# wbuntine/libstb

Hardware: AMD Instinct MI355X
Metric: S-table cells/s (higher is better)
Workload: dtype f64

## Files before the change

### include/stb_hip.h

```cpp
#ifndef STB_HIP_H
#define STB_HIP_H

#include <stddef.h>
#include <stdint.h>

#ifdef __cplusplus
extern "C" {
#endif

const char *stb_last_error(void);
int stb_device_count(void);
int stb_device_name(char *buf, int len);

int stb_set_device(int dev);
int stb_get_device(void);
int stb_device_enter(int dev);
void stb_device_leave(int prev);

void *stb_device_malloc(size_t bytes);
void stb_device_free(void *p);
void *stb_host_malloc(size_t bytes);
void stb_host_free(void *p);
void *stb_host_malloc_huge(size_t bytes);
void stb_host_free_huge(void *p);
// ... 16 lines not shown
uint64_t stb_vrowoff(unsigned n, unsigned M);

void stb_extend_policy(unsigned usedN, unsigned usedM, unsigned maxN, unsigned maxM, int N, int M,
                       unsigned *newN, unsigned *newM);

#define STB_FILL_SCALED 0
#define STB_FILL_LOGDOMAIN 1
#define STB_FILL_SCALED_STEP 2
#define STB_FILL_SPLIT 3
#define STB_FILL_FUSED 4
#define STB_FILL_PC 5
#define STB_FILL_CHAIN 6
#define STB_FILL_CHAINX 7
#define STB_FILL_CK 8
#define STB_FILL_HB 9
size_t stb_fill_workspace_bytes(unsigned N, unsigned M, int D);
int stb_default_variant(void);
int stb_fill_S(const double *a_host, int D, unsigned N, unsigned M, double *d_tables,
               uint64_t table_stride, double *d_S1, uint64_t s1_stride, void *d_ws, size_t ws_bytes,
               int variant, void *stream);
int stb_fill_tuning(unsigned N, unsigned M, int D, int *C_out, int *R_out, int *launches);
int stb_fill_status(void);
unsigned stb_fill_fallbacks(void);
unsigned stb_slow_launches(void);
int stb_shared_gpu_mode(void);
void stb_set_shared_gpu(int mode);
void stb_note_launch_span(double span_ms, double expect_ms);
int stb_has_ablation(void);
void stb_pool_trim(void);
void stb_fill_profile_begin(void);
int stb_fill_profile_end(double *kernel_ms_total, int *launches);
double stb_fill_profile_span(void);
int stb_fill_V(const double *a_host, int D, unsigned N, unsigned M, double *d_vtables,
               uint64_t vtable_stride, void *d_ws, size_t ws_bytes, void *stream);
int stb_fill_V_exact(const double *a_host, int D, unsigned N, unsigned M, double *d_vtables,
                     uint64_t vtable_stride, void *d_ws, size_t ws_bytes, void *stream);

int stb_fill_takes_kind(unsigned N, unsigned M, int D, int kind);
int stb_fill_Sf(const double *a_host, int D, unsigned N, unsigned M, float *d_tables, uint64_t table_stride,
                double *d_S1, uint64_t s1_stride, void *d_ws, size_t ws_bytes, void *stream);
int stb_fill_Vf(const double *a_host, int D, unsigned N, unsigned M, float *d_vtables, uint64_t vtable_stride,
                void *d_ws, size_t ws_bytes, void *stream);

int stb_table_to_float(const double *d_src, float *d_dst, uint64_t elems, void *stream);

int stb_lookup_S(const double *d_table, const double *d_S1, unsigned N, unsigned M,
// ... 120 lines not shown
```

### libstb_amd/capi.py

```python
from __future__ import annotations

import ctypes as C
import os
from functools import lru_cache

import numpy as np

_HERE = os.path.dirname(os.path.abspath(__file__))
LIB_PATH = os.environ.get("STB_LIB_PATH") or os.path.join(_HERE, "lib", "libstb_amd.so")

S_STABLE, S_UVTABLE, S_FLOAT, S_VERBOSE, S_QUITONBOUND, S_THREADS, S_ASYMPT = 1, 2, 4, 8, 16, 32, 64
FILL_SCALED, FILL_LOGDOMAIN, FILL_SCALED_STEP, FILL_SPLIT, FILL_FUSED, FILL_PC, FILL_CHAIN, FILL_CHAINX, FILL_CK, FILL_HB = 0, 1, 2, 3, 4, 5, 6, 7, 8, 9

c_double_p = C.POINTER(C.c_double)
c_u32_p = C.POINTER(C.c_uint32)
c_u16_p = C.POINTER(C.c_uint16)
c_int_p = C.POINTER(C.c_int)
c_float_p = C.POINTER(C.c_float)

LOGDENS = C.CFUNCTYPE(C.c_double, C.c_double, C.c_void_p)
GETVAL = C.CFUNCTYPE(None, c_u32_p, c_u16_p, C.c_uint, C.c_uint)


class StbError(RuntimeError):
    pass


@lru_cache(maxsize=None)
def lib() -> C.CDLL:
    if not os.path.exists(LIB_PATH):
        raise StbError(
            f"{LIB_PATH} is missing: build it with `python -c 'import __graft_entry__ as g; g.build()'` "
            "or `make -C libstb_amd/csrc` (there is no pure-Python or CPU implementation)")
    try:
        import torch
    except Exception:
        pass
    L = C.CDLL(LIB_PATH)
    u, d, i, vp, u64, sz = C.c_uint, C.c_double, C.c_int, C.c_void_p, C.c_uint64, C.c_size_t

    ROUND5 = {"stb_groups_pairs_begin", "stb_groups_pairs_put", "stb_groups_pairs_put_ragged", "stb_groups_pairs_commit",
              "stb_groups_update_pairs", "stb_groups_fallbacks", "stb_grid_shape", "stb_bterms_update",
              "stb_table_probe", "stb_slow_launches", "stb_shared_gpu_mode", "stb_set_shared_gpu", "stb_note_launch_span",
              "stb_lookup_V", "stb_lookup_U", "stb_lookup_UV", "stb_groups_aterms_multi", "stb_groups_create_node",
              "stb_groups_last_form"}

    def sig(name, res, args):
        try:
            f = getattr(L, name)
        except AttributeError:
            if name in ROUND5 and os.environ.get("STB_LIB_PATH"):
                return
            raise
        f.restype = res
        f.argtypes = args

    sig("S_make", vp, [u, u, u, u, d, C.c_uint32])
    sig("S_tag", None, [vp, C.c_char_p])
    sig("S_remake", i, [vp, d])
    sig("S_free", None, [vp])
    for n in ("S_S", "S_U", "S_UV", "S_V", "S_asympt"):
        sig(n, d, [vp, u, u])
    sig("S_S1", d, [vp, u])
    sig("S_report", None, [vp, vp])
    sig("stb_extend_policy", None, [u, u, u, u, i, i, C.POINTER(u), C.POINTER(u)])
    sig("stb_table_sync", i, [vp])
    sig("stb_table_probe", None, [vp, i, C.POINTER(u), C.POINTER(u), sz, c_double_p])
    sig("stb_table_mirrored", None, [vp, C.POINTER(u), C.POINTER(u)])
# ... 3 lines not shown
    sig("stb_device_count", i, [])
    sig("stb_device_name", i, [C.c_char_p, i])
    sig("stb_set_device", i, [i])
    sig("stb_get_device", i, [])
    sig("stb_device_enter", i, [i])
    sig("stb_device_leave", None, [i])
    sig("stb_device_malloc", vp, [sz])
    sig("stb_device_free", None, [vp])
    sig("stb_host_malloc", vp, [sz])
    sig("stb_host_free", None, [vp])
    sig("stb_memcpy_h2d", i, [vp, vp, sz, vp])
    sig("stb_memcpy_d2h", i, [vp, vp, sz, vp])
    sig("stb_stream_sync", i, [vp])
    for n in ("stb_cells", "stb_elems", "stb_vcells", "stb_velems"):
        sig(n, u64, [u, u])
    sig("stb_rowoff", u64, [u, u])
    sig("stb_vrowoff", u64, [u, u])
    sig("stb_fill_workspace_bytes", sz, [u, u, i])
    sig("stb_default_variant", i, [])
    sig("stb_fill_S", i, [c_double_p, i, u, u, vp, u64, vp, u64, vp, sz, i, vp])
    sig("stb_fill_tuning", i, [u, u, i, c_int_p, c_int_p, c_int_p])
    sig("stb_fill_status", i, [])
    sig("stb_fill_fallbacks", C.c_uint, [])
    sig("stb_has_ablation", i, [])
    sig("stb_slow_launches", C.c_uint, [])
    sig("stb_shared_gpu_mode", i, [])
    sig("stb_set_shared_gpu", None, [i])
    sig("stb_note_launch_span", None, [C.c_double, C.c_double])
    sig("stb_fill_profile_begin", None, [])
    sig("stb_fill_profile_end", i, [c_double_p, c_int_p])
    sig("stb_fill_profile_span", C.c_double, [])
    sig("stb_fill_V", i, [c_double_p, i, u, u, vp, u64, vp, sz, vp])
    sig("stb_fill_V_exact", i, [c_double_p, i, u, u, vp, u64, vp, sz, vp])
    sig("stb_fill_Vf", i, [c_double_p, i, u, u, vp, u64, vp, sz, vp])
    sig("stb_fill_Sf", i, [c_double_p, i, u, u, vp, u64, vp, u64, vp, sz, vp])
    sig("stb_fill_takes_kind", i, [u, u, i, i])
    sig("stb_bterms_create", vp, [c_u32_p, i])
    sig("stb_bterms_update", i, [vp, c_u32_p, i])
    sig("stb_bterms_eval", i, [vp, c_double_p, i, d, d, d, c_double_p])
    sig("stb_bterms_free", None, [vp])
    sig("stb_table_to_float", i, [vp, vp, u64, vp])
    sig("stb_lookup_S", i, [vp, vp, u, u, vp, vp, u64, vp, vp])
    sig("stb_lookup_V", i, [vp, u, u, vp, vp, u64, vp, vp])
    sig("stb_lookup_U", i, [vp, u, u, C.c_double, vp, vp, u64, vp, vp])
    sig("stb_lookup_UV", i, [vp, u, u, C.c_double, vp, vp, u64, vp, vp])
    sig("stb_sweep_workspace_bytes", sz, [u64, i])
# ... 525 lines not shown
```

### libstb_amd/csrc/abi.hip

```cpp

#include <mutex>
#include <vector>

#include "stb_common.h"


static thread_local char g_err[512] = "";

int stb_fail(const char *fmt, ...) {
  va_list ap;
  va_start(ap, fmt);
  vsnprintf(g_err, sizeof(g_err), fmt, ap);
  va_end(ap);
  return 1;
}

extern "C" const char *stb_last_error(void) { return g_err; }

#include <atomic>
static std::atomic<unsigned> g_slow_launches{0};
static std::atomic<int> g_shared_mode{-2};
extern "C" void yaps_message(const char *fmt, ...);

static int shared_mode_now() {
// ... 221 lines not shown
  }
  if (release >= 0) pool_raw_free(p, release);
  return known;
}

extern "C" void stb_pool_trim(void) {
  STB_ENTRY;
  std::vector<pool_block> drop;
  {
    std::lock_guard<std::mutex> lk(g_pool_mu);
    for (size_t i = 0; i < g_pool.size();) {
      if (!g_pool[i].used) {
        drop.push_back(g_pool[i]);
        g_pool.erase(g_pool.begin() + i);
      } else {
        i++;
      }
    }
    g_pool_idle[0] = g_pool_idle[1] = 0;
  }
  for (const pool_block &q : drop) pool_raw_free(q.p, q.kind);
}

extern "C" void *stb_device_malloc(size_t bytes) {
  STB_ENTRY;
  void *p = nullptr;
  hipError_t e = stb_pool_malloc(&p, bytes ? bytes : 1, 0);
  if (e != hipSuccess) {
    stb_fail("hipMalloc(%zu) failed: %s", bytes, hipGetErrorString(e));
    (void)hipGetLastError();
    return nullptr;
  }
  return p;
}
extern "C" void stb_device_free(void *p) {
  STB_ENTRY;
  if (p && !stb_pool_free(p)) (void)hipFree(p);
}
extern "C" void *stb_host_malloc(size_t bytes) {
  STB_ENTRY;
  void *p = nullptr;
  hipError_t e = stb_pool_malloc(&p, bytes ? bytes : 1, 1);
  if (e != hipSuccess) {
    stb_fail("hipHostMalloc(%zu) failed: %s", bytes, hipGetErrorString(e));
    (void)hipGetLastError();
    return nullptr;
// ... 121 lines not shown
```

### libstb_amd/csrc/fill.hip

```cpp

#include "stb_common.h"

static unsigned frontier_pitch(unsigned M) { return (unsigned)stb_align_up((size_t)M + 2, 64); }

int stb_period_rows(unsigned N) {
  int bits = 1;
  while ((1ull << bits) < (unsigned long long)N) bits++;
  const int p = 1450 / (2 * bits + 1);
  return p < 1 ? 1 : p;
}

struct fill_prof {
  bool armed = false;
  int used = 0;
  hipEvent_t ev[2 * 4096];
  int made = 0;
  double span_ms = 0.0;
};
static thread_local fill_prof g_prof;

void stb_prof_events(hipEvent_t *e0, hipEvent_t *e1) {
  *e0 = *e1 = nullptr;
  if (!g_prof.armed || g_prof.used + 2 > 2 * 4096) return;
  while (g_prof.made < g_prof.used + 2) {
// ... 174 lines not shown
  A.H = 256 - 64 * ncw;
  A.R = stb_env_int("STB_FILL_R", A.H);
  if (A.R > A.H) A.R = A.H;
  if (A.R < 1) A.R = 1;
  A.Wv = 256 - A.H;
}

void stb_fill_last(last_fill *out) { *out = g_last; }

int stb_fill_status_of(last_fill *lf) {
  if (!lf->hdr) return 0;
  unsigned h[10] = {0, 0, 0, 0, 0, 0, 0, 0, 0, 0};
  HIPCHK(hipMemcpyAsync(h, lf->hdr, lf->stamped ? sizeof(h) : 4 * sizeof(unsigned), hipMemcpyDeviceToHost, lf->st));
  HIPCHK(hipStreamSynchronize(lf->st));
  if (lf->stamped) {
    const unsigned long long t0 = (unsigned long long)h[STB_HDR_T0] | ((unsigned long long)h[STB_HDR_T0 + 1] << 32);
    const unsigned long long t1 = (unsigned long long)h[STB_HDR_T1] | ((unsigned long long)h[STB_HDR_T1 + 1] << 32);
    if (t0 && t1 > t0)
      stb_note_span((double)(t1 - t0) * 1e-5, 1e-3 * (100.0 + 0.05 * (double)lf->A.N * (1.0 + (double)lf->D / 8.0)), "a table fill (stb_fill_S)");
  }
  if (h[1] == 0) return 0;
  stb_fail("%s: the fill gave up waiting for a neighbour block (code 0x%x, block %u of table %u)",
           lf->s_table ? "stb_fill_S" : "stb_fill_V", h[1], h[2] & 0xffffu, h[2] >> 16);
  if (!lf->can_fall_back || stb_env_int("STB_CHAIN_NO_FALLBACK", 0)) {
    lf->hdr = nullptr;
    return 1;
  }
  lf->hdr = nullptr;
  lf->fell_back = true;
  g_fallbacks++;
  fill_args A = lf->A;
  pc_geometry(A);
  if (stb_launch_pc(A, lf->D, lf->st)) return 1;
  HIPCHK(hipStreamSynchronize(lf->st));
  return 0;
}

extern "C" int stb_fill_status(void) {
  STB_ENTRY;
  return stb_fill_status_of(&g_last);
}

static bool hb_takes_kind(unsigned N, unsigned M, int D, int kind) {
  if (stb_env_int("STB_HB", -1) == 0 || stb_shared_gpu() || !stb_hb_eligible_out(N, M, D, kind)) return false;
  const uint64_t cells = (uint64_t)D * stb_table_cells(N, M);
  if (N < (unsigned)stb_env_int("STB_HB_MIN_N", 512) || cells > (uint64_t)stb_env_int("STB_HB_MAX_MCELLS", 1250) * 1000000ull) return false;
// ... 17 lines not shown
  *D_out = g_a_D;
  g_a_D = 0;
  return true;
}
int stb_a_flush(const fill_args &A, hipStream_t st) {
  stb_a64 av;
  int D = 0;
  if (!stb_a_take(&av, &D)) return 0;
  hipLaunchKernelGGL(k_set_a, dim3(1), dim3(64), 0, st, av, const_cast<double *>(A.a), D);
  HIPCHK(hipGetLastError());
  return 0;
}

static thread_local bool g_fillv_exact = false;

static int fill_common(const double *a_host, int D, unsigned N, unsigned M, double *d_tables, uint64_t table_stride,
                       double *d_S1, uint64_t s1_stride, void *d_ws, size_t ws_bytes, int variant, int kind,
                       hipStream_t st) {
  const bool vtable = (kind & 2) != 0;
  const char *who = vtable ? "stb_fill_V" : "stb_fill_S";
  g_last.hdr = nullptr;
  g_last.fell_back = false;
  g_last.stamped = false;
  struct a_guard {
    a_guard() { g_a_D = 0; }
    ~a_guard() { g_a_D = 0; }
  } a_guard_;
  if (D < 1) return stb_fail("%s: D=%d", who, D);
  if (N < 2 || M < 2) return stb_fail("%s: bounds N=%u M=%u too small", who, N, M);
  if (!a_host || !d_tables || !d_ws || (!vtable && !d_S1)) return stb_fail("%s: null pointer", who);
  if (ws_bytes < fill_workspace_need(N, M, D))
    return stb_fail("%s: workspace %zu < %zu", who, ws_bytes, fill_workspace_need(N, M, D));
  const uint64_t need = vtable ? stb_vtable_elems(N, M) : stb_table_elems(N, M);
  if (table_stride < need || (!vtable && s1_stride < N)) return stb_fail("%s: strides too small", who);
  if (D > 1 && (table_stride & 1)) return stb_fail("%s: table stride must be even", who);
  for (int d = 0; d < D; d++)
    if (!(a_host[d] >= 0.0 && a_host[d] < 1.0)) return stb_fail("%s: discount %g outside [0,1)", who, a_host[d]);

  fill_args A;
  memset(&A, 0, sizeof(A));
  char *ws = (char *)d_ws;
  A.a = (const double *)ws;
  ws += stb_align_up((size_t)D * sizeof(double), 256);
  A.W = frontier_pitch(M);
  A.fm = (double *)ws;
  A.fe = (int *)(ws + (size_t)D * 2 * A.W * sizeof(double));
  ws = (char *)d_ws + ws_head(M, D);
  const size_t ws_left = ws_bytes - ws_head(M, D);
  A.tables = d_tables;
  A.tstride = table_stride;
  A.S1 = d_S1;
  A.s1stride = s1_stride;
  A.N = N;
  A.M = M;
  if (stb_logtab(&A.lt)) return 1;
  if (D <= 64 && stb_env_int("STB_A_BY_VALUE", 1)) {
    stb_a_defer(a_host, D);
  } else {
    HIPCHK(hipMemcpyAsync((void *)A.a, a_host, (size_t)D * sizeof(double), hipMemcpyHostToDevice, st));
  }

  if (kind != 0 && !(kind == 2 && (g_fillv_exact || stb_env_int("STB_FILLV_EXACT", 0) || !hb_takes_kind(N, M, D, kind)))) {
    if (!hb_takes_kind(N, M, D, kind))
      return stb_fail("%s: no kernel stores %s for N=%u M=%u D=%d (the caller narrows a double table instead)", who,
                      kind == 1 ? "floats" : (kind == 2 ? "V ratios" : "float V ratios"), N, M, D);
    unsigned *hdr = nullptr;
    if (stb_launch_hb(A, D, ws, ws_left, nullptr, &hdr, st, kind)) return 1;
    g_last.hdr = hdr;
    g_last.stamped = true;
    g_last.A = A;
    g_last.D = D;
    g_last.st = st;
    g_last.s_table = !vtable;
    g_last.can_fall_back = false;
    return 0;
  }
  if (vtable) {
    if (stb_a_flush(A, st)) return 1;
    if (stb_env_int("STB_FILLV_CHAIN", 1) && !stb_shared_gpu()) {
      unsigned *hdr = nullptr;
      if (stb_launch_vchain(A, D, ws, ws_left, &hdr, st)) return 1;
      g_last.hdr = hdr;
      g_last.st = st;
      g_last.s_table = false;
      g_last.can_fall_back = false;
      return 0;
    }
    const int C = 2;
    A.R = stb_env_int("STB_FILL_R", 48);
    if (A.R < 1) A.R = 1;
// ... 14 lines not shown
      g_last.hdr = hdr;
      g_last.A = A;
      g_last.D = D;
      g_last.st = st;
      g_last.s_table = true;
      g_last.can_fall_back = (g_dot_req == nullptr);
      return 0;
    }
    case FORM_CK: {
      unsigned *hdr = nullptr;
      if (stb_launch_ck(A, D, ws, ws_left, g_dot_req, &hdr, st)) return 1;
      g_last.hdr = hdr;
      g_last.A = A;
      g_last.D = D;
      g_last.st = st;
      g_last.s_table = true;
      g_last.can_fall_back = (g_dot_req == nullptr);
      return 0;
    }
    case FORM_HB: {
      unsigned *hdr = nullptr;
      if (g_dot_req && g_dot_req->col0 == 4) {
        if (stb_launch_grid(A, D, ws, ws_left, g_dot_req, &hdr, st)) return 1;
      } else if (stb_launch_hb(A, D, ws, ws_left, g_dot_req, &hdr, st)) return 1;
      g_last.hdr = hdr;
      g_last.stamped = !(g_dot_req && g_dot_req->col0 == 4);
      g_last.A = A;
      g_last.D = D;
      g_last.st = st;
      g_last.s_table = true;
      g_last.can_fall_back = (g_dot_req == nullptr);
      return 0;
    }
    case FORM_PC:
      pc_geometry(A);
      return stb_launch_pc(A, D, st);
    case FORM_ROWS_LOG: {
      const bool few = (uint64_t)D * M < 40000;
      int C = stb_env_int("STB_FILL_C", few ? 1 : 2);
      if (C != 1 && C != 2 && C != 4) return stb_fail("STB_FILL_C must be 1, 2 or 4");
      A.R = stb_env_int("STB_FILL_R", few ? 48 : 64);
      if (A.R < 1) A.R = 1;
      A.H = (A.R + C - 1) / C * C;
      if (A.H > 64 * C - C) return stb_fail("STB_FILL_R=%d too large for C=%d", A.R, C);
      A.Wv = 64 * C - A.H;
      return stb_launch_rows(A, D, C, STB_ROWS_LOGDOM, st);
    }
// ... 53 lines not shown
```

### libstb_amd/csrc/fill_hb.hip

```cpp

#include <algorithm>
#include <mutex>
#include <type_traits>
#include <vector>

#include "fill_chain.h"

#ifndef HB_NW
#define HB_NW 8
#endif
#define HB_PMAX 7
#define HB_SLOTS 8
#define HB_FSLOTS 8
#define HB_MAXHL 32
__host__ __device__ constexpr int hb_mhl(int C) { return C == 1 ? HB_MAXHL : (C == 2 ? 25 : (C == 3 ? 17 : 13)); }
#ifndef HB_NW_DOT4
#define HB_NW_DOT4 14
#endif
#define HB_EOFF32 (1u << 30)
#define HB_WRITTEN 0x8000000000000000ull
#define HB_DOT_GR 8
#define HB_DOT_NQ 6
#define HB_MAXCNT 64
#define HB_CNT0 64
// ... 21 lines not shown
  unsigned *progress;
  const unsigned *order;
  const unsigned *rec_off;
  unsigned n_rec;
  int D, B, JW, NB;
  int P, R, HL, U;
  unsigned n_tiles;
  unsigned n_order;
  int split;
  unsigned n_spine;
  unsigned long long timeout;
  int poll_nap;
  int nap_block;
  int diag;
  int n_cnt;
  int order_lds;
  int spare_work;
  int doze;
  const unsigned *item_ptr;
  const unsigned short *ent_pos;
  const unsigned *ent_cnt;
  double *dotp;
  unsigned long long *dbg;
};

typedef double hb_double2 __attribute__((ext_vector_type(2)));

__device__ __forceinline__ void hb_store16(const void *sbase, unsigned byte_off, double x, double y) {
  unsigned long long base_copy;
  hb_double2 v2 = {x, y};
  asm volatile("s_mov_b64 %0, %3\n\tglobal_store_dwordx4 %1, %2, %0\n\ts_nop 1"
               : "=&s"(base_copy)
               : "v"(byte_off), "v"(v2), "s"(sbase)
               : "memory");
}

__device__ __forceinline__ void hb_store_wt16(unsigned long long *p, unsigned long long a, unsigned long long b) {
  typedef unsigned long long hb_u64x2 __attribute__((ext_vector_type(2)));
  const hb_u64x2 v2 = {a, b};
  asm volatile("global_store_dwordx4 %0, %1, off sc1\n\ts_nop 1" ::"v"(p), "v"(v2) : "memory");
}

template <int C>
__device__ __forceinline__ void hb_store_record(unsigned long long mask, unsigned long long *p, const double (&v)[C]) {
  typedef unsigned long long hb_u64x2 __attribute__((ext_vector_type(2)));
  unsigned long long saved;
// ... 122 lines not shown
  const int tid = threadIdx.x, lane = tid & 63;
  const int wave = __builtin_amdgcn_readfirstlane(tid >> 6);
  if (tid == 0) s_ticket = atomicAdd(X.hdr, 1u);
  if constexpr (LTX) {
    for (int i = tid; i < 128 * 16; i += blockDim.x) lt[i] = A.lt[i >> 4];
  } else {
    if (tid < 128) lt[tid] = A.lt[tid];
  }
  const bool order_in_lds = X.order_lds != 0;
  if (order_in_lds)
    for (unsigned i = tid; i < X.n_order; i += blockDim.x) s_order[i] = X.order[i];
  for (int i = tid; i < HB_MAXCNT; i += blockDim.x) s_done[i] = 0;
  const bool recoff_in_lds = X.JW + 2 <= HB_RECOFF_LDS;
  if (recoff_in_lds)
    for (int i = tid; i < X.JW + 2; i += blockDim.x) s_recoff[i] = X.rec_off[i];
  __syncthreads();
  auto rec_off = [&](int sidx) -> unsigned { return recoff_in_lds ? s_recoff[sidx] : X.rec_off[sidx]; };
  const unsigned ticket = s_ticket;
  const unsigned N = A.N, M = A.M;
  const int R = X.R, HL = X.HL, U = X.U, NB = X.NB, P = X.P;
  const int UC = U * C;
  if (ticket == 0 && tid == 0)
    __hip_atomic_store(reinterpret_cast<unsigned long long *>(X.hdr + STB_HDR_T0), (unsigned long long)wall_clock64(), __ATOMIC_RELAXED, __HIP_MEMORY_SCOPE_AGENT);

  if (ticket < X.n_spine) {
    const int j = (int)(ticket / (unsigned)X.D);
    const int d = (int)(ticket % (unsigned)X.D);
    const int jw0 = j * P;
    if (tid < HB_NW) {
      const int jw = jw0 + tid;
      const int b0 = (jw < X.JW) ? hb_first_block(jw, UC, R) : NB;
      c_posted[tid + 1] = b0;
      c_taken[tid] = b0;
    }
    if (tid == 0) {
      c_posted[0] = hb_first_block(jw0, UC, R);
      c_taken[HB_NW] = 0x7fffffff;
      c_huge = 0x7fffffff;
      c_never = -0x7fffffff;
      s_abort = 0;
      s_awake = (j == 0) ? 1 : 0;
    }
    __syncthreads();
    const unsigned who = (unsigned)(j | (d << 16));
    bool aborted = false;
    auto wait_ge = [&](const int *cnt, int need, unsigned code) {
      if (aborted) return;
      for (int k = 0; k < HB_SPIN; k++) {
        if (lds_peek(cnt) >= need) {
          asm volatile("" ::: "memory");
          return;
        }
        __builtin_amdgcn_s_sleep(1);
      }
      if (!chain_wait_slow(cnt, need, &s_abort, X.hdr, X.timeout, code, who, 1)) aborted = true;
      asm volatile("" ::: "memory");
    };
    const size_t tab_rec = (size_t)d * X.n_rec;

    if (wave < P) {
      const int w = wave;
      const int jw = jw0 + w;
      if (jw < X.JW) {
        const int b0 = hb_first_block(jw, UC, R);
        const double a = A.a[d];
        const int m0 = 2 + (jw * U - HL + lane) * C;
        double v[C], coef[C];
#pragma unroll
        for (int i = 0; i < C; i++) {
          v[i] = 0.0;
          coef[i] = (double)(1 + b0 * R) - (double)(m0 + i) * a;
        }
        int ep = 1 + PC_BIAS + (int)HB_EB;
        if (jw == 0 && lane == HL - 1) v[C - 1] = ldexp(1.0, -1 - PC_BIAS);
        const bool has_next = (w + 1 < P) && (jw + 1 < X.JW);
        const int *left_cnt = &c_posted[w];
        unsigned long long *dbg = (X.dbg && d == 0 && lane == 0) ? X.dbg + (size_t)jw * (NB + 2) : nullptr;
        const bool own = lane >= HL;
        const size_t rec_base = own ? tab_rec + rec_off(jw + 1) - (size_t)b0 : tab_rec + rec_off(0);
        const int slot = own ? lane - HL : lane + U - HL;
        unsigned long long *rec_v = X.ck_v + (rec_base * U + slot) * C;
        unsigned *rec_e = X.ck_e + rec_base * U + slot;
        unsigned *prog = X.progress + ((size_t)d * X.JW + jw) * HB_PROG_STRIDE;
        double s = 1.0;
#ifdef HB_TL_FINE
        unsigned long long *fdbg = dbg ? X.dbg + (size_t)X.JW * (NB + 2) + (size_t)X.n_order * 4 + (size_t)jw * NB * 8 : nullptr;
#ifndef HB_FINE_SET
#define HB_FINE_SET 0x7f
// ... 344 lines not shown
        __builtin_amdgcn_s_sleep(64);
    } else if (wave > P || (wave == P && j == 0) || (wave < P && jw0 + wave >= X.JW)) {
      const int last = min(P, X.JW - jw0) - 1;
      unsigned spins = 0;
      while (__hip_atomic_load(X.progress + ((size_t)d * X.JW + jw0 + last) * HB_PROG_STRIDE, __ATOMIC_RELAXED, __HIP_MEMORY_SCOPE_AGENT) != 0x7fffffffu &&
             !lds_peek(&s_abort)) {
        __builtin_amdgcn_s_sleep(127);
        if ((++spins & 1023u) == 0 && __hip_atomic_load(X.hdr + 1, __ATOMIC_RELAXED, __HIP_MEMORY_SCOPE_AGENT) != 0) break;
      }
    }
    if (__hip_atomic_load(X.hdr, __ATOMIC_RELAXED, __HIP_MEMORY_SCOPE_AGENT) < gridDim.x) return;
  }

  {
    int one_hi = 0x3ff00000;
    asm volatile("" : "+v"(one_hi));
    if (X.diag & 1) {
      unsigned spins = 0;
      while (__hip_atomic_load(X.hdr + 4, __ATOMIC_RELAXED, __HIP_MEMORY_SCOPE_AGENT) < (unsigned)(X.JW * X.D) && ++spins < 400000u)
        __builtin_amdgcn_s_sleep(100);
    }
    const unsigned NC = (unsigned)X.n_cnt, Dg = min((unsigned)X.D, (unsigned)HB_MAXCNT), S = NC / Dg;
    unsigned cur = ((unsigned)blockIdx.x * NW + (unsigned)wave) % NC, misses = 0;
    for (;;) {
      if (lds_peek(&s_done[cur])) {
        if (++misses >= NC) break;
        cur = (cur + 1 == NC) ? 0 : cur + 1;
        continue;
      }
      const unsigned grp = cur % Dg, part = cur / Dg;
      const unsigned Tg = ((unsigned)X.D - grp + Dg - 1) / Dg;
      const unsigned mine = (X.n_order + S - 1 - part) / S * Tg;
      unsigned k = 0;
      if (lane == 0) k = atomicAdd(X.hdr + HB_CNT0 + cur * HB_PROG_STRIDE, 1u);
      k = (unsigned)__builtin_amdgcn_readfirstlane((int)k);
      if (k >= mine) {
        if (lane == 0) __hip_atomic_store(&s_done[cur], 1, __ATOMIC_RELAXED, __HIP_MEMORY_SCOPE_WORKGROUP);
        if (++misses >= NC) break;
        cur = (cur + 1 == NC) ? 0 : cur + 1;
        continue;
      }
      misses = 0;
      const int d = (int)(grp + Dg * (k % Tg));
      const unsigned oi = (k / Tg) * S + part;
      const unsigned ord = (unsigned)__builtin_amdgcn_readfirstlane((int)(order_in_lds ? s_order[oi] : X.order[oi]));
      const int jw = (int)(ord & (X.split ? 0x3fffu : 0xffffu)), b = (int)(ord >> 16);
// ... 81 lines not shown
                __hip_atomic_store(X.hdr + 1, 0xA00u, __ATOMIC_RELAXED, __HIP_MEMORY_SCOPE_AGENT);
              }
              ok = false;
              break;
            }
          }
          if (!ok) break;
          __builtin_amdgcn_s_sleep(8);
          if ((++tries & 63u) != 0 && X.timeout != 0) continue;
          if (t_begin == 0) t_begin = wall_clock64();
          const unsigned err = __hip_atomic_load(X.hdr + 1, __ATOMIC_RELAXED, __HIP_MEMORY_SCOPE_AGENT);
          if (err != 0 || (unsigned long long)wall_clock64() - t_begin >= X.timeout) {
            if (err == 0 && lane == 0) {
              __hip_atomic_store(X.hdr + 2, who, __ATOMIC_RELAXED, __HIP_MEMORY_SCOPE_AGENT);
              __hip_atomic_store(X.hdr + 1, 0xA00u, __ATOMIC_RELAXED, __HIP_MEMORY_SCOPE_AGENT);
            }
            ok = false;
            break;
          }
        }
      }
      if (!ok) break;
      if (wdbg) wdbg[1] = wall_clock64();
      const double a = A.a[d];
      const int mE0 = 2 + (jw * U - HL) * C;
      const double n1 = (double)(1 + b * R);
#pragma unroll
      for (int g = 0; g < NG; g++) {
        const int m0 = mE0 + ((NG == 2) ? g * 128 + 2 * lane : lane * C);
#pragma unroll
        for (int i = 0; i < CG; i++) coef[g][i] = n1 - (double)(m0 + i) * a;
      }
      double s[NG], z1 = 0.0;
#pragma unroll
      for (int g = 0; g < NG; g++) {
        const int dl = wave_shr1(ep[g], ep[g]) - ep[g];
        s[g] = (lane == 0) ? 0.0 : ldexp(1.0, min(max(dl, -1100), 220));
      }
      if constexpr (NG == 2) {
        const int e63 = __builtin_amdgcn_readlane(ep[0], 63);
        if (lane == 0) z1 = ldexp(1.0, min(max(e63 - ep[1], -1100), 220));
      }
      if constexpr (DOT != 0) {
        constexpr int WS = 64 * C;
        double *stage = hb_dyn + (size_t)wave * (4 * WS);
        int *se = &w_se[DOT ? wave : 0][0];
#pragma unroll
// ... 167 lines not shown
                if (own[0]) hb_store16(rp, voff, val[u * 2], val[u * 2 + 1]);
              } else {
                if (own[0]) hb_store16(rp, voff, val[u * 4], val[u * 4 + 1]);
                if (own[1]) hb_store16(rp + 128, voff, val[u * 4 + 2], val[u * 4 + 3]);
              }
            }
            roff += rpitch(nu);
          }
        } else {
#pragma unroll
          for (int u = 0; u < RS; u++) roff += rpitch(n + u);
        }
        n += RS;
      }
      }
      if (wdbg) {
        unsigned hw, xcc;
        asm volatile("s_getreg_b32 %0, hwreg(HW_REG_HW_ID)" : "=s"(hw));
        asm volatile("s_getreg_b32 %0, hwreg(HW_REG_XCC_ID)" : "=s"(xcc));
        wdbg[2] = wall_clock64();
        wdbg[3] = (unsigned long long)hw | ((unsigned long long)(xcc & 15u) << 32);
      }
    }
  }
}


struct hb_geom {
  int C, P, B, JW, NB, R, HL, U;
  unsigned n_tiles, n_rec;
  size_t off_prog, off_cke, off_ckv, zero_bytes, bytes;
  bool ok;
};

int stb_cu_count() {
  int dev = 0, cus = 256;
  if (hipGetDevice(&dev) != hipSuccess || hipDeviceGetAttribute(&cus, hipDeviceAttributeMultiprocessorCount, dev) != hipSuccess || cus < 1)
    cus = 256;
  return cus;
}

static hb_geom hb_geometry(unsigned N, unsigned M, int D, int sum_C = 0, bool vt = false) {
  const bool summing = sum_C != 0;
  hb_geom g;
  memset(&g, 0, sizeof(g));
  g.ok = false;
// ... 202 lines not shown
  return (c == 2 || c == 3) ? c : 4;
}

int stb_hb_dot_info(unsigned N, unsigned M, int D, hb_dot_info *out, int sum_C) {
  const hb_geom g = hb_geometry(N, M, D, (sum_C == 2 || sum_C == 3) ? sum_C : 4);
  if (!g.ok || g.R % HB_DOT_GR != 0 || g.R / HB_DOT_GR > HB_DOT_NQ) return 1;
  const unsigned *rec_off = nullptr, *order = nullptr;
  if (hb_order_list(g, N, M, &rec_off, &order)) return 1;
  out->R = g.R;
  out->UC = g.U * g.C;
  out->HC = g.HL * g.C;
  out->NB = g.NB;
  out->JW = g.JW;
  out->NQ = HB_DOT_NQ;
  out->G = HB_DOT_GR;
  out->C = g.C;
  out->n_tiles = g.n_tiles;
  out->n_rec = g.n_rec;
  out->n_spine = (unsigned)g.B * (unsigned)D;
  out->rec_off = rec_off;
  return 0;
}

int stb_launch_hb(fill_args &A, int D, char *ws, size_t ws_left, const dot_request *dot, unsigned **hdr_out, hipStream_t st, int out_kind) {
  const unsigned N = A.N, M = A.M;
  if (out_kind < 0 || out_kind > 3 || (out_kind && dot)) return stb_fail("stb_fill: output kind %d", out_kind);
  const hb_geom g = hb_geometry(N, M, D, dot ? ((dot->geom_C == 2 || dot->geom_C == 3) ? dot->geom_C : 4) : 0, (out_kind & 2) != 0);
  if (!g.ok) return stb_fail("stb_fill_S: the halo-block form does not take N=%u M=%u D=%d", N, M, D);
  if (g.bytes > ws_left) return stb_fail("stb_fill_S: workspace too small for the halo-block form (%zu > %zu)", g.bytes, ws_left);
  if (dot && (!dot->item_ptr || dot->col0 != 3))
    return stb_fail("stb_fill_S: the halo-block form sums over cell lists built for its tiles");
  if (dot && (g.R % HB_DOT_GR != 0 || g.R / HB_DOT_GR > HB_DOT_NQ)) return stb_fail("stb_fill_S: blocks of %d rows do not suit the summing form", g.R);
  hb_args X;
  memset(&X, 0, sizeof(X));
  X.hdr = (unsigned *)ws;
  X.progress = (unsigned *)(ws + g.off_prog);
  X.ck_e = (unsigned *)(ws + g.off_cke);
  X.ck_v = (unsigned long long *)(ws + g.off_ckv);
  X.n_rec = g.n_rec;
  X.D = D;
  X.B = g.B;
  X.JW = g.JW;
  X.NB = g.NB;
  X.P = g.P;
  X.R = g.R;
  X.HL = g.HL;
  X.U = g.U;
  X.n_tiles = g.n_tiles;
  X.n_spine = (unsigned)g.B * (unsigned)D;
  X.timeout = (unsigned long long)stb_env_int("STB_CHAIN_TIMEOUT_MS", 2000) * 100000ull;
  X.poll_nap = stb_env_int("STB_HB_POLL_NAP", 4);
  if (X.poll_nap < 1) X.poll_nap = 1;
  X.nap_block = stb_env_int("STB_HB_NAP_BLOCK", g.C >= 3 ? (dot ? 6 : 4) : 3);
  X.diag = stb_env_int("STB_HB_DIAG", 0);
  X.spare_work = stb_env_int("STB_HB_SPARE", dot ? 64 : 0);
  X.doze = stb_env_int("STB_HB_DOZE", 0);
  if (dot) {
    X.item_ptr = dot->item_ptr;
    X.ent_pos = dot->ent_pos;
    X.ent_cnt = dot->ent_cnt;
    X.dotp = dot->dotp;
    const_cast<dot_request *>(dot)->parts_per_table = (int)g.n_tiles;
    if (dot->dotp_cap && (size_t)D * g.n_tiles > dot->dotp_cap) return stb_fail("stb_groups_aterms: partial-sum buffer too small");
  }
  X.split = (!dot && g.R == 48 && g.C >= 2 && g.JW < (1 << 14)) ? std::min(stb_env_int("STB_HB_SPLIT", g.C == 2 ? 6 : 0), g.NB) : 0;
  if (X.split < 0) X.split = 0;
  X.n_order = g.n_tiles;
  if (hb_order_list(g, N, M, &X.rec_off, &X.order, X.split, &X.n_order)) return 1;
  const char *tl_file = getenv("STB_HB_TIMELINE");
#ifdef HB_TL_FINE
  const size_t dbg_words = (size_t)g.JW * (g.NB + 2) + (size_t)X.n_order * 4 + (size_t)g.JW * g.NB * 8 + (size_t)g.JW * g.NB * 2;
#else
  const size_t dbg_words = (size_t)g.JW * (g.NB + 2) + (size_t)X.n_order * 4;
#endif
  if (tl_file && *tl_file) {
    HIPCHK(hipMalloc((void **)&X.dbg, dbg_words * 8));
    HIPCHK(hipMemsetAsync(X.dbg, 0, dbg_words * 8, st));
  }
  {
    const bool need_zero = !dot || dot->ws_zero < g.zero_bytes;
    const bool need_s1 = !(dot && dot->no_s1) && !(out_kind & 2);
    if (need_zero && need_s1 && !(g.zero_bytes & 15) && !((uintptr_t)ws & 15) && stb_env_int("STB_HB_PREP", 1)) {
      if (stb_launch_prep(A, D, ws, g.zero_bytes, st)) return 1;
    } else {
      if (stb_a_flush(A, st)) return 1;
      if (need_zero) HIPCHK(hipMemsetAsync(ws, 0, g.zero_bytes, st));
      if (need_s1 && stb_launch_s1(A, D, st)) return 1;
    }
  }
  if (dot) const_cast<dot_request *>(dot)->zero_bytes = g.zero_bytes;
  *hdr_out = X.hdr;
  const int cus = stb_cu_count();
  const int per_cu = stb_env_int("STB_HB_WG_PER_CU", 1);
  unsigned grid = (unsigned)(cus * per_cu);
  const unsigned min_workers = (unsigned)stb_env_int("STB_HB_MIN_WORKERS", 48);
  if (dot) {
    const uint64_t fed = (uint64_t)D * N / 250;
    const uint64_t want = (uint64_t)X.n_spine + (fed > min_workers ? fed : min_workers);
    if (want < grid) grid = (unsigned)want;
  }
  if (grid < X.n_spine + min_workers) grid = X.n_spine + min_workers;
  if (stb_env_int("STB_HB_GRID", 0) > 0) grid = (unsigned)stb_env_int("STB_HB_GRID", 0);
  X.order_lds = (!dot && X.n_order <= HB_ORDER_LDS) ? 1 : 0;
  {
    const int Dg = D < HB_MAXCNT ? D : HB_MAXCNT;
    int Sn = stb_env_int("STB_HB_TICKET_PARTS", Dg >= 8 ? 1 : (8 + Dg - 1) / Dg);
    while (Sn > 1 && ((unsigned)Sn * 64 > X.n_order || Sn * Dg > HB_MAXCNT)) Sn--;
    if (Sn < 1) Sn = 1;
    X.n_cnt = Sn * Dg;
  }
  if (X.n_cnt < 1 || X.n_cnt > HB_MAXCNT) return stb_fail("stb_fill_S: %d ticket counters", X.n_cnt);
  if (dot) {
    const int nw = g.C >= 3 ? HB_NW_DOT4 : HB_NW;
    const size_t shm = (size_t)nw * 4 * 64 * g.C * sizeof(double);
    switch (g.C) {
      case 4: STB_LAUNCH_SHM((k_fill_hb<4, 1>), dim3(grid), dim3(64 * nw), shm, st, A, X); break;
      case 3: STB_LAUNCH_SHM((k_fill_hb<3, 1>), dim3(grid), dim3(64 * nw), shm, st, A, X); break;
      case 2: STB_LAUNCH_SHM((k_fill_hb<2, 1>), dim3(grid), dim3(64 * HB_NW), shm, st, A, X); break;
      default: return stb_fail("stb_fill_S: no summing halo-block kernel for %d columns per lane", g.C);
    }
  } else {
    const size_t shm = X.order_lds ? (size_t)X.n_order * sizeof(unsigned) : 0;
    if (out_kind && g.C == 1) return stb_fail("stb_fill: the halo-block form narrows or divides with 2 or 4 columns per lane");
    switch (g.C * 4 + out_kind) {
      case 4: STB_LAUNCH_SHM((k_fill_hb<1, 0>), dim3(grid), dim3(64 * HB_NW), shm, st, A, X); break;
      case 8: STB_LAUNCH_SHM((k_fill_hb<2, 0>), dim3(grid), dim3(64 * HB_NW), shm, st, A, X); break;
      case 9: STB_LAUNCH_SHM((k_fill_hb<2, 0, 1>), dim3(grid), dim3(64 * HB_NW), shm, st, A, X); break;
      case 10: STB_LAUNCH_SHM((k_fill_hb<2, 0, 2>), dim3(grid), dim3(64 * HB_NW), shm, st, A, X); break;
      case 11: STB_LAUNCH_SHM((k_fill_hb<2, 0, 3>), dim3(grid), dim3(64 * HB_NW), shm, st, A, X); break;
      case 16: STB_LAUNCH_SHM((k_fill_hb<4, 0>), dim3(grid), dim3(64 * HB_NW), shm, st, A, X); break;
      case 17: STB_LAUNCH_SHM((k_fill_hb<4, 0, 1>), dim3(grid), dim3(64 * HB_NW), shm, st, A, X); break;
      case 18: STB_LAUNCH_SHM((k_fill_hb<4, 0, 2>), dim3(grid), dim3(64 * HB_NW), shm, st, A, X); break;
      default: STB_LAUNCH_SHM((k_fill_hb<4, 0, 3>), dim3(grid), dim3(64 * HB_NW), shm, st, A, X); break;
    }
  }
  HIPCHK(hipGetLastError());
  if (X.dbg) {
    HIPCHK(hipStreamSynchronize(st));
    std::vector<unsigned long long> h(dbg_words);
    HIPCHK(hipMemcpy(h.data(), X.dbg, dbg_words * 8, hipMemcpyDeviceToHost));
    (void)hipFree(X.dbg);
    FILE *f = fopen(tl_file, "wb");
    if (f) {
      const int hd[8] = {g.JW, g.NB, (int)X.n_order, g.C, g.P, g.R, g.U, D | (X.split << 16)};
      fwrite(hd, sizeof(int), 8, f);
      std::vector<unsigned> ord(X.n_order);
      HIPCHK(hipMemcpy(ord.data(), X.order, (size_t)X.n_order * sizeof(unsigned), hipMemcpyDeviceToHost));
      fwrite(ord.data(), sizeof(unsigned), X.n_order, f);
      fwrite(h.data(), 8, dbg_words, f);
      fclose(f);
    }
  }
  return 0;
}
```

### libstb_amd/csrc/stb_common.h

```cpp
#ifndef STB_COMMON_H
#define STB_COMMON_H

#include <hip/hip_runtime.h>
#include <hip/hip_ext.h>

#include <cmath>
#include <cstdarg>
#include <cstdint>
#include <cstdio>
#include <cstdlib>
#include <cstring>

#include "stb_layout.h"
#include "../../include/stb_hip.h"


int stb_fail(const char *fmt, ...);

#define HIPCHK(expr)                                                                       \
  do {                                                                                     \
    hipError_t e_ = (expr);                                                                \
    if (e_ != hipSuccess)                                                                  \
      return stb_fail("%s failed: %s (%s:%d)", #expr, hipGetErrorString(e_), __FILE__, __LINE__); \
  } while (0)

struct stb_rand_guard {
  stb_rand_guard();
  ~stb_rand_guard();
  stb_rand_guard(const stb_rand_guard &) = delete;
  stb_rand_guard &operator=(const stb_rand_guard &) = delete;
};
#define STB_ENTRY stb_rand_guard stb_rand_guard_

hipError_t stb_pool_malloc(void **out, size_t bytes, int kind = 0);
bool stb_pool_free(void *p);

int stb_use_device(void);

int stb_logtab(const double2 **out);

static inline size_t stb_align_up(size_t x, size_t a) { return (x + a - 1) / a * a; }
static inline int stb_env_int(const char *name, int dflt) {
  const char *s = getenv(name);
  if (!s || !*s) return dflt;
  return atoi(s);
}


struct fill_args {
  const double *a;
  double *tables;
  uint64_t tstride;
  double *S1;
  uint64_t s1stride;
  double *fm;
  int *fe;
  const double2 *lt;
  unsigned W;
  unsigned N, M;
  int R;
  int H;
  int Wv;
};

struct last_fill {
  unsigned *hdr = nullptr;
  fill_args A;
  int D = 0;
  bool s_table = false, can_fall_back = false;
  bool fell_back = false;
  bool stamped = false;
  hipStream_t st = nullptr;
};
void stb_fill_last(last_fill *out);
int stb_fill_status_of(last_fill *lf);

void stb_prof_events(hipEvent_t *e0, hipEvent_t *e1);
#define STB_LAUNCH_SHM(KERN, GRID, BLOCK, SHM, ST, ...)                                 \
  do {                                                                                  \
    hipEvent_t pe0_ = nullptr, pe1_ = nullptr;                                          \
    stb_prof_events(&pe0_, &pe1_);                                                      \
    if (pe0_)                                                                           \
      hipExtLaunchKernelGGL(KERN, GRID, BLOCK, SHM, ST, pe0_, pe1_, 0, __VA_ARGS__);    \
    else                                                                                \
      hipLaunchKernelGGL(KERN, GRID, BLOCK, SHM, ST, __VA_ARGS__);                      \
  } while (0)
#define STB_LAUNCH(KERN, GRID, BLOCK, ST, ...) STB_LAUNCH_SHM(KERN, GRID, BLOCK, 0, ST, __VA_ARGS__)

int stb_period_rows(unsigned N);

bool stb_shared_gpu();
void stb_note_span(double span_ms, double expect_ms, const char *what);
#define STB_HDR_T0 6
#define STB_HDR_T1 8

// ... 18 lines not shown
  size_t zero_bytes = 0;
  int no_s1 = 0;
};
void stb_set_dot_request(const dot_request *r);
size_t stb_chain_workspace(unsigned N, unsigned M, int D);
int stb_launch_chain(fill_args &A, int D, char *ws, size_t ws_left, const dot_request *dot, unsigned **hdr_out,
                     hipStream_t st);
int stb_launch_vchain(fill_args &A, int D, char *ws, size_t ws_left, unsigned **hdr_out, hipStream_t st);
int stb_chain_tuning(unsigned N, unsigned M, int D, int *W_out);
bool stb_ck_eligible(unsigned N, unsigned M, int D) __attribute__((weak));
size_t stb_ck_workspace(unsigned N, unsigned M, int D) __attribute__((weak));
int stb_ck_tuning(unsigned N, unsigned M, int D, int *W_out, int *rows_out) __attribute__((weak));
int stb_launch_ck(fill_args &A, int D, char *ws, size_t ws_left, const dot_request *dot, unsigned **hdr_out, hipStream_t st)
    __attribute__((weak));
unsigned stb_ck_dot_parts(unsigned N, unsigned M, int D) __attribute__((weak));
unsigned stb_ck_dot_spine(unsigned N, unsigned M, int D) __attribute__((weak));

int stb_cu_count();
bool stb_hb_eligible(unsigned N, unsigned M, int D);
bool stb_hb_eligible_out(unsigned N, unsigned M, int D, int out_kind);
size_t stb_hb_workspace(unsigned N, unsigned M, int D);
unsigned stb_hb_spine(unsigned N, unsigned M, int D);
int stb_hb_tuning(unsigned N, unsigned M, int D, int *W_out, int *rows_out);
int stb_launch_hb(fill_args &A, int D, char *ws, size_t ws_left, const dot_request *dot, unsigned **hdr_out, hipStream_t st, int out_kind = 0);
struct hb_dot_info {
  int R, UC, HC, NB, JW, NQ;
  int G, C;
  unsigned n_tiles, n_rec, n_spine;
  const unsigned *rec_off;
};
int stb_hb_sum_C(unsigned N, unsigned M, int Dmax);
int stb_hb_dot_info(unsigned N, unsigned M, int D, hb_dot_info *out, int sum_C);

struct grid_geom {
  int C, P, B, JW, NB, R, HL, U;
  int G, NQ, phases;
  int K;
  unsigned n_tiles;
  unsigned job_cap;
  size_t off_cke, off_ckv, off_state_e, off_state_v, zero_bytes, bytes;
  size_t off_jflag, off_jrec_e, off_jrec_v;
  int ok;
};
int stb_grid_geometry(unsigned N, unsigned M, int D, grid_geom *out);
size_t stb_grid_workspace(unsigned N, unsigned M, int D);
unsigned stb_grid_job_cap(int C, int D, unsigned n_tiles, int phases);
int stb_launch_grid(fill_args &A, int D, char *ws, size_t ws_left, const dot_request *dot, unsigned **hdr_out, hipStream_t st);
// ... 119 lines not shown
```

Before: 220.8 billion.

## Double-buffer HB fill workspace so kernel pre-zeroes the next call's records

Adds per-stream, library-owned double-buffered record workspaces for the halo-block fill. Each fill's idle worker threads zero the other half while it runs, so the next call can skip the separate prep/memset launch. The discount vector is also passed in the kernel arguments and written by the kernel, and the S1 launch moves behind the main kernel, leaving the fill as effectively one launch. In exchange it holds extra device memory per stream, adds mutex-guarded bookkeeping and possible device syncs on eviction, and risks stale state if a fill aborts, which is handled by marking the buffers dirty.

```diff
diff --git a/include/stb_hip.h b/include/stb_hip.h
--- a/include/stb_hip.h
+++ b/include/stb_hip.h
@@ -62,6 +62,9 @@
 int stb_fill_tuning(unsigned N, unsigned M, int D, int *C_out, int *R_out, int *launches);
 int stb_fill_status(void);
 unsigned stb_fill_fallbacks(void);
+unsigned long long stb_hb_one_launch_fills(void);
+unsigned long long stb_hb_storing_fills(void);
+unsigned stb_own_pairs(void);
 unsigned stb_slow_launches(void);
 int stb_shared_gpu_mode(void);
 void stb_set_shared_gpu(int mode);
diff --git a/libstb_amd/capi.py b/libstb_amd/capi.py
--- a/libstb_amd/capi.py
+++ b/libstb_amd/capi.py
@@ -43,7 +43,8 @@
               "stb_groups_update_pairs", "stb_groups_fallbacks", "stb_grid_shape", "stb_bterms_update",
               "stb_table_probe", "stb_slow_launches", "stb_shared_gpu_mode", "stb_set_shared_gpu", "stb_note_launch_span",
               "stb_lookup_V", "stb_lookup_U", "stb_lookup_UV", "stb_groups_aterms_multi", "stb_groups_create_node",
-              "stb_groups_last_form"}
+              "stb_groups_last_form",
+              "stb_hb_one_launch_fills", "stb_hb_storing_fills", "stb_own_pairs"}
 
     def sig(name, res, args):
         try:
@@ -93,6 +94,9 @@
     sig("stb_fill_tuning", i, [u, u, i, c_int_p, c_int_p, c_int_p])
     sig("stb_fill_status", i, [])
     sig("stb_fill_fallbacks", C.c_uint, [])
+    sig("stb_hb_one_launch_fills", C.c_ulonglong, [])
+    sig("stb_hb_storing_fills", C.c_ulonglong, [])
+    sig("stb_own_pairs", C.c_uint, [])
     sig("stb_has_ablation", i, [])
     sig("stb_slow_launches", C.c_uint, [])
     sig("stb_shared_gpu_mode", i, [])
diff --git a/libstb_amd/csrc/abi.hip b/libstb_amd/csrc/abi.hip
--- a/libstb_amd/csrc/abi.hip
+++ b/libstb_amd/csrc/abi.hip
@@ -1,4 +1,5 @@
 
+#include <algorithm>
 #include <mutex>
 #include <vector>
 
@@ -267,6 +268,128 @@
   for (const pool_block &q : drop) pool_raw_free(q.p, q.kind);
 }
 
+struct own_pair {
+  unsigned long long id;
+  int dev;
+  hipStream_t st;
+  const void *ws;
+  char *buf[2];
+  size_t cap;
+  size_t clean[2];
+  int next;
+  unsigned long long used;
+};
+static std::mutex g_own_mu;
+static std::vector<own_pair> g_own;
+static unsigned long long g_own_lookups = 0, g_own_ids = 0;
+
+static void own_release(own_pair &p) {
+  for (int h = 0; h < 2; h++) {
+    if (p.buf[h] && !stb_pool_free(p.buf[h])) (void)hipFree(p.buf[h]);
+    p.buf[h] = nullptr;
+    p.clean[h] = 0;
+  }
+  p.cap = 0;
+}
+static bool own_alloc(own_pair &p, size_t bytes) {
+  const size_t cap = stb_align_up(bytes, 4096);
+  for (int h = 0; h < 2; h++) {
+    void *q = nullptr;
+    if (stb_pool_malloc(&q, cap, 0) != hipSuccess) {
+      (void)hipGetLastError();
+      own_release(p);
+      return false;
+    }
+    p.buf[h] = (char *)q;
+    p.clean[h] = 0;
+  }
+  p.cap = cap;
+  p.next = 0;
+  return true;
+}
+
+bool stb_own_take(hipStream_t st, const void *ws, size_t bytes, stb_own_lease *out) {
+  const size_t half_max = (size_t)std::max(stb_env_int("STB_HB_OWN_MB", 128), 0) << 20;
+  const size_t pairs_max = (size_t)std::max(stb_env_int("STB_HB_OWN_PAIRS", 16), 0);
+  if (bytes == 0 || bytes > half_max || pairs_max == 0) return false;
+  int dev = 0;
+  if (hipGetDevice(&dev) != hipSuccess) {
+    (void)hipGetLastError();
+    return false;
+  }
+  std::lock_guard<std::mutex> lk(g_own_mu);
+  g_own_lookups++;
+  own_pair *p = nullptr;
+  for (own_pair &q : g_own)
+    if (q.dev == dev && q.st == st && q.ws == ws) p = &q;
+  if (p && p->cap < bytes) {
+    if (hipStreamSynchronize(st) != hipSuccess) {
+      (void)hipGetLastError();
+      return false;
+    }
+    own_release(*p);
+    if (!own_alloc(*p, bytes)) {
+      g_own.erase(g_own.begin() + (p - g_own.data()));
+      return false;
+    }
+  }
+  if (!p) {
+    while (g_own.size() >= pairs_max) {
+      size_t old = g_own.size();
+      for (size_t i = 0; i < g_own.size(); i++)
+        if (g_own[i].used + 32 < g_own_lookups && (old == g_own.size() || g_own[i].used < g_own[old].used)) old = i;
+      if (old == g_own.size()) return false;
+      const int cur = dev;
+      const bool there = g_own[old].dev == cur || hipSetDevice(g_own[old].dev) == hipSuccess;
+      const bool idle = there && hipDeviceSynchronize() == hipSuccess;
+      if (g_own[old].dev != cur) (void)hipSetDevice(cur);
+      if (!idle) {
+        (void)hipGetLastError();
+        return false;
+      }
+      own_release(g_own[old]);
+      g_own.erase(g_own.begin() + (long)old);
+    }
+    own_pair q;
+    memset(&q, 0, sizeof(q));
+    q.id = ++g_own_ids;
+    q.dev = dev;
+    q.st = st;
+    q.ws = ws;
+    if (!own_alloc(q, bytes)) return false;
+    g_own.push_back(q);
+    p = &g_own.back();
+  }
+  p->used = g_own_lookups;
+  out->id = p->id;
+  out->half = p->next;
+  out->use = p->buf[p->next];
+  out->use_clean = p->clean[p->next];
+  out->other = p->buf[p->next ^ 1];
+  p->clean[p->next] = 0;
+  return true;
+}
+
+void stb_own_commit(const stb_own_lease &l, size_t other_clean) {
+  std::lock_guard<std::mutex> lk(g_own_mu);
+  for (own_pair &q : g_own)
+    if (q.id == l.id && q.buf[l.half] == l.use) {
+      q.clean[l.half ^ 1] = other_clean;
+      q.next = l.half ^ 1;
+    }
+}
+
+void stb_own_dirty(unsigned long long id) {
+  std::lock_guard<std::mutex> lk(g_own_mu);
+  for (own_pair &q : g_own)
+    if (q.id == id) q.clean[0] = q.clean[1] = 0;
+}
+
+extern "C" unsigned stb_own_pairs(void) {
+  std::lock_guard<std::mutex> lk(g_own_mu);
+  return (unsigned)g_own.size();
+}
+
 extern "C" void *stb_device_malloc(size_t bytes) {
   STB_ENTRY;
   void *p = nullptr;
diff --git a/libstb_amd/csrc/fill.hip b/libstb_amd/csrc/fill.hip
--- a/libstb_amd/csrc/fill.hip
+++ b/libstb_amd/csrc/fill.hip
@@ -220,6 +220,7 @@
   if (h[1] == 0) return 0;
   stb_fail("%s: the fill gave up waiting for a neighbour block (code 0x%x, block %u of table %u)",
            lf->s_table ? "stb_fill_S" : "stb_fill_V", h[1], h[2] & 0xffffu, h[2] >> 16);
+  if (lf->own) stb_own_dirty(lf->own);
   if (!lf->can_fall_back || stb_env_int("STB_CHAIN_NO_FALLBACK", 0)) {
     lf->hdr = nullptr;
     return 1;
@@ -283,6 +284,7 @@
   g_last.hdr = nullptr;
   g_last.fell_back = false;
   g_last.stamped = false;
+  g_last.own = 0;
   struct a_guard {
     a_guard() { g_a_D = 0; }
     ~a_guard() { g_a_D = 0; }
@@ -326,7 +328,7 @@
       return stb_fail("%s: no kernel stores %s for N=%u M=%u D=%d (the caller narrows a double table instead)", who,
                       kind == 1 ? "floats" : (kind == 2 ? "V ratios" : "float V ratios"), N, M, D);
     unsigned *hdr = nullptr;
-    if (stb_launch_hb(A, D, ws, ws_left, nullptr, &hdr, st, kind)) return 1;
+    if (stb_launch_hb(A, D, ws, ws_left, nullptr, &hdr, st, kind, &g_last.own)) return 1;
     g_last.hdr = hdr;
     g_last.stamped = true;
     g_last.A = A;
@@ -387,7 +389,7 @@
       unsigned *hdr = nullptr;
       if (g_dot_req && g_dot_req->col0 == 4) {
         if (stb_launch_grid(A, D, ws, ws_left, g_dot_req, &hdr, st)) return 1;
-      } else if (stb_launch_hb(A, D, ws, ws_left, g_dot_req, &hdr, st)) return 1;
+      } else if (stb_launch_hb(A, D, ws, ws_left, g_dot_req, &hdr, st, 0, &g_last.own)) return 1;
       g_last.hdr = hdr;
       g_last.stamped = !(g_dot_req && g_dot_req->col0 == 4);
       g_last.A = A;
diff --git a/libstb_amd/csrc/fill_hb.hip b/libstb_amd/csrc/fill_hb.hip
--- a/libstb_amd/csrc/fill_hb.hip
+++ b/libstb_amd/csrc/fill_hb.hip
@@ -1,5 +1,6 @@
 
 #include <algorithm>
+#include <atomic>
 #include <mutex>
 #include <type_traits>
 #include <vector>
@@ -67,6 +68,11 @@
   const unsigned *ent_cnt;
   double *dotp;
   unsigned long long *dbg;
+  uint4 *clean;
+  unsigned long long clean_n16;
+  int clean_late;
+  int Da;
+  stb_a64 av;
 };
 
 typedef double hb_double2 __attribute__((ext_vector_type(2)));
@@ -235,6 +241,7 @@
   const int UC = U * C;
   if (ticket == 0 && tid == 0)
     __hip_atomic_store(reinterpret_cast<unsigned long long *>(X.hdr + STB_HDR_T0), (unsigned long long)wall_clock64(), __ATOMIC_RELAXED, __HIP_MEMORY_SCOPE_AGENT);
+  if (ticket == 0 && tid < X.Da) const_cast<double *>(A.a)[tid] = X.av.v[tid];
 
   if (ticket < X.n_spine) {
     const int j = (int)(ticket / (unsigned)X.D);
@@ -276,7 +283,7 @@
       const int jw = jw0 + w;
       if (jw < X.JW) {
         const int b0 = hb_first_block(jw, UC, R);
-        const double a = A.a[d];
+        const double a = X.Da > 0 ? X.av.v[d] : A.a[d];
         const int m0 = 2 + (jw * U - HL + lane) * C;
         double v[C], coef[C];
 #pragma unroll
@@ -667,6 +674,13 @@
     }
     const unsigned NC = (unsigned)X.n_cnt, Dg = min((unsigned)X.D, (unsigned)HB_MAXCNT), S = NC / Dg;
     unsigned cur = ((unsigned)blockIdx.x * NW + (unsigned)wave) % NC, misses = 0;
+    auto clean_other = [&]() {
+      if (X.clean_n16 == 0 || ticket < X.n_spine) return;
+      const unsigned long long nthr = (unsigned long long)(gridDim.x - X.n_spine) * blockDim.x;
+      const uint4 z = {0u, 0u, 0u, 0u};
+      for (unsigned long long i = (unsigned long long)(ticket - X.n_spine) * blockDim.x + tid; i < X.clean_n16; i += nthr) X.clean[i] = z;
+    };
+    if (!X.clean_late) clean_other();
     for (;;) {
       if (lds_peek(&s_done[cur])) {
         if (++misses >= NC) break;
@@ -794,7 +808,7 @@
       }
       if (!ok) break;
       if (wdbg) wdbg[1] = wall_clock64();
-      const double a = A.a[d];
+      const double a = X.Da > 0 ? X.av.v[d] : A.a[d];
       const int mE0 = 2 + (jw * U - HL) * C;
       const double n1 = (double)(1 + b * R);
 #pragma unroll
@@ -1008,6 +1022,7 @@
         wdbg[3] = (unsigned long long)hw | ((unsigned long long)(xcc & 15u) << 32);
       }
     }
+    if (X.clean_late) clean_other();
   }
 }
 
@@ -1256,8 +1271,14 @@
   return 0;
 }
 
-int stb_launch_hb(fill_args &A, int D, char *ws, size_t ws_left, const dot_request *dot, unsigned **hdr_out, hipStream_t st, int out_kind) {
+static std::atomic<unsigned long long> g_hb_one_launch{0}, g_hb_storing{0};
+extern "C" unsigned long long stb_hb_one_launch_fills(void) { return g_hb_one_launch.load(); }
+extern "C" unsigned long long stb_hb_storing_fills(void) { return g_hb_storing.load(); }
+
+int stb_launch_hb(fill_args &A, int D, char *ws, size_t ws_left, const dot_request *dot, unsigned **hdr_out, hipStream_t st, int out_kind,
+                  unsigned long long *own_out) {
   const unsigned N = A.N, M = A.M;
+  if (own_out) *own_out = 0;
   if (out_kind < 0 || out_kind > 3 || (out_kind && dot)) return stb_fail("stb_fill: output kind %d", out_kind);
   const hb_geom g = hb_geometry(N, M, D, dot ? ((dot->geom_C == 2 || dot->geom_C == 3) ? dot->geom_C : 4) : 0, (out_kind & 2) != 0);
   if (!g.ok) return stb_fail("stb_fill_S: the halo-block form does not take N=%u M=%u D=%d", N, M, D);
@@ -1267,10 +1288,13 @@
   if (dot && (g.R % HB_DOT_GR != 0 || g.R / HB_DOT_GR > HB_DOT_NQ)) return stb_fail("stb_fill_S: blocks of %d rows do not suit the summing form", g.R);
   hb_args X;
   memset(&X, 0, sizeof(X));
-  X.hdr = (unsigned *)ws;
-  X.progress = (unsigned *)(ws + g.off_prog);
-  X.ck_e = (unsigned *)(ws + g.off_cke);
-  X.ck_v = (unsigned long long *)(ws + g.off_ckv);
+  stb_own_lease own;
+  const bool owned = !dot && !(g.zero_bytes & 15) && stb_env_int("STB_HB_ONE_LAUNCH", 1) != 0 && stb_own_take(st, ws, g.zero_bytes, &own);
+  char *rec = owned ? own.use : ws;
+  X.hdr = (unsigned *)rec;
+  X.progress = (unsigned *)(rec + g.off_prog);
+  X.ck_e = (unsigned *)(rec + g.off_cke);
+  X.ck_v = (unsigned long long *)(rec + g.off_ckv);
   X.n_rec = g.n_rec;
   X.D = D;
   X.B = g.B;
@@ -1311,16 +1335,18 @@
     HIPCHK(hipMalloc((void **)&X.dbg, dbg_words * 8));
     HIPCHK(hipMemsetAsync(X.dbg, 0, dbg_words * 8, st));
   }
-  {
-    const bool need_zero = !dot || dot->ws_zero < g.zero_bytes;
-    const bool need_s1 = !(dot && dot->no_s1) && !(out_kind & 2);
-    if (need_zero && need_s1 && !(g.zero_bytes & 15) && !((uintptr_t)ws & 15) && stb_env_int("STB_HB_PREP", 1)) {
-      if (stb_launch_prep(A, D, ws, g.zero_bytes, st)) return 1;
-    } else {
-      if (stb_a_flush(A, st)) return 1;
-      if (need_zero) HIPCHK(hipMemsetAsync(ws, 0, g.zero_bytes, st));
-      if (need_s1 && stb_launch_s1(A, D, st)) return 1;
-    }
+  const bool need_zero = owned ? own.use_clean < g.zero_bytes : (!dot || dot->ws_zero < g.zero_bytes);
+  const bool need_s1 = !(dot && dot->no_s1) && !(out_kind & 2);
+  const bool s1_behind = owned && !need_zero && need_s1;
+  if (owned && !need_zero) {
+    if (!stb_a_take(&X.av, &X.Da)) X.Da = 0;
+    if (X.Da != 0 && X.Da != D) return stb_fail("stb_fill: %d discounts on their way, %d tables", X.Da, D);
+  } else if (need_zero && need_s1 && !(g.zero_bytes & 15) && !((uintptr_t)rec & 15) && stb_env_int("STB_HB_PREP", 1)) {
+    if (stb_launch_prep(A, D, rec, g.zero_bytes, st)) return 1;
+  } else {
+    if (stb_a_flush(A, st)) return 1;
+    if (need_zero) HIPCHK(hipMemsetAsync(rec, 0, g.zero_bytes, st));
+    if (need_s1 && stb_launch_s1(A, D, st)) return 1;
   }
   if (dot) const_cast<dot_request *>(dot)->zero_bytes = g.zero_bytes;
   *hdr_out = X.hdr;
@@ -1335,6 +1361,11 @@
   }
   if (grid < X.n_spine + min_workers) grid = X.n_spine + min_workers;
   if (stb_env_int("STB_HB_GRID", 0) > 0) grid = (unsigned)stb_env_int("STB_HB_GRID", 0);
+  if (owned && grid > X.n_spine) {
+    X.clean = (uint4 *)own.other;
+    X.clean_n16 = g.zero_bytes / 16;
+    X.clean_late = stb_env_int("STB_HB_CLEAN_LATE", 1) != 0;
+  }
   X.order_lds = (!dot && X.n_order <= HB_ORDER_LDS) ? 1 : 0;
   {
     const int Dg = D < HB_MAXCNT ? D : HB_MAXCNT;
@@ -1369,6 +1400,15 @@
     }
   }
   HIPCHK(hipGetLastError());
+  if (s1_behind && stb_launch_s1(A, D, st)) return 1;
+  if (owned) {
+    stb_own_commit(own, X.clean_n16 * 16);
+    if (own_out) *own_out = own.id;
+  }
+  if (!dot) {
+    g_hb_storing++;
+    if (owned && !need_zero) g_hb_one_launch++;
+  }
   if (X.dbg) {
     HIPCHK(hipStreamSynchronize(st));
     std::vector<unsigned long long> h(dbg_words);
diff --git a/libstb_amd/csrc/stb_common.h b/libstb_amd/csrc/stb_common.h
--- a/libstb_amd/csrc/stb_common.h
+++ b/libstb_amd/csrc/stb_common.h
@@ -34,6 +34,17 @@
 
 hipError_t stb_pool_malloc(void **out, size_t bytes, int kind = 0);
 bool stb_pool_free(void *p);
+
+struct stb_own_lease {
+  unsigned long long id = 0;
+  int half = 0;
+  char *use = nullptr;
+  size_t use_clean = 0;
+  char *other = nullptr;
+};
+bool stb_own_take(hipStream_t st, const void *ws, size_t bytes, stb_own_lease *out);
+void stb_own_commit(const stb_own_lease &l, size_t other_clean);
+void stb_own_dirty(unsigned long long id);
 
 int stb_use_device(void);
 
@@ -71,6 +82,7 @@
   bool fell_back = false;
   bool stamped = false;
   hipStream_t st = nullptr;
+  unsigned long long own = 0;
 };
 void stb_fill_last(last_fill *out);
 int stb_fill_status_of(last_fill *lf);
@@ -135,7 +147,8 @@
 size_t stb_hb_workspace(unsigned N, unsigned M, int D);
 unsigned stb_hb_spine(unsigned N, unsigned M, int D);
 int stb_hb_tuning(unsigned N, unsigned M, int D, int *W_out, int *rows_out);
-int stb_launch_hb(fill_args &A, int D, char *ws, size_t ws_left, const dot_request *dot, unsigned **hdr_out, hipStream_t st, int out_kind = 0);
+int stb_launch_hb(fill_args &A, int D, char *ws, size_t ws_left, const dot_request *dot, unsigned **hdr_out, hipStream_t st, int out_kind = 0,
+                  unsigned long long *own_out = nullptr);
 struct hb_dot_info {
   int R, UC, HC, NB, JW, NQ;
   int G, C;
```

New measurement: 217.7 billion. -1.4%, worse.
